# anonymous-author-918/deq-mpc-corl

Hardware: AMD Instinct MI355X
Metric: QP solves/sec at (B,T=20,nx=13,nu=4) (higher is better)
Workload: dtype f32

## Files before the change

### deq-mpc-corl_amd/csrc/alqp_quad.hip

```cpp
#include <hip/hip_runtime.h>

#include "alqp_quad.hpp"
#include "alqp_dims.hpp"
#include "alqp_launch.hpp"

#if defined(ALQP_QUAD_F32) == defined(ALQP_QUAD_F64)
#error "compile alqp_quad.hip with exactly one of -DALQP_QUAD_F32, -DALQP_QUAD_F64"
#endif

namespace alqp {

#ifndef ALQP_FUSE_LS
#define ALQP_FUSE_LS 1
#endif
#ifdef ALQP_PHASE_TIMING
__device__ unsigned long long g_phase_cycles[10];
#define QSTAMP(b) qd.stamp(b)
#else
#define QSTAMP(b)
#endif
template <typename real, int NX, int NU, bool TRACE, class Dyn = NoDyn>
__global__ __launch_bounds__(64) __attribute__((amdgpu_waves_per_eu(1, 1))) void k_solve_lin_quad(SolveArgs<real> a, TraceArgs<real> tr, real *ws) {
    using C = QCfg<real, NX, NU>;
    constexpr bool NL = Dyn::ID != 0;
// ... 19 lines not shown
            if (mode == 4) simd = (simd & 1) ^ (blockIdx.x & 1);
            if (mode == 5) simd = (hw >> 8) & 3;
            for (int i = 0; i < simd * stag; ++i) __builtin_amdgcn_s_sleep(16);
        }
    }
#ifdef ALQP_ALIAS_ALL
    const int b = (active ? b_raw : a.B - 1) % ALQP_ALIAS_ALL;
#else
    const int b = active ? b_raw : a.B - 1;
#endif
    const int T = a.T, M = C::M(T);

    Quad<real, NX, NU> qd;
    __shared__ real w_lds[QCfg<real, NX, NU>::WLDS_WORDS];
    qd.wl = w_lds + threadIdx.x;
    qd.q = lane & 3;
    qd.T = T;
    qd.active = active;
    qd.gQd = a.Qd + (size_t)b * T * N;
    qd.gq = a.q + (size_t)b * T * N;
    qd.gF = a.F + (size_t)b * (T - 1) * NX * N;
    qd.gc = a.c + (size_t)b * (T - 1) * NX;
    qd.gx0 = a.x0 + (size_t)b * NX;
    qd.gulo = a.ulo + (size_t)b * a.sb_u;
    qd.guhi = a.uhi + (size_t)b * a.sb_u;
    qd.st_u = a.st_u;
    qd.gz = a.z + (size_t)b * T * N;
    qd.glam = a.lam + (size_t)b * M;
    qd.rec = ws + C::rec_base(b, T);
    qd.gFw = const_cast<real *>(qd.gF);
    qd.dyn_h = a.dyn_h;
    qd.rho = a.rho[b];
    qd.info = 0;
    real phi_prev = a.phi[b];
#ifdef ALQP_PHASE_TIMING
    for (int i = 0; i < 10; ++i) qd.tacc[i] = 0;
#endif
    QSTAMP(-1);
    if (!(a.flags & ALQP_WS_PRIMED)) {
        if constexpr (NL) qd.stage_in(false, false);
        else qd.stage_in(a.max_newton == 0 || a.al_iter == 0 || (a.flags & ALQP_EXIT_IN_KERNEL) ||
                         (!C::PHI0_FWD && (a.flags & ALQP_INIT_MERIT)));
    }
    const bool ref_exit = (a.flags & ALQP_EXIT_IN_KERNEL) != 0;
    int gphase = 0;

    int step_id = 0;
    bool pend = false;
    real alpha_pend = 0;
    int bad = 0;
    real rn2 = 0, phi_next = 0;
    for (int it = 0; it < a.al_iter; ++it) {
        bool phi_from_forward = false;
        if (a.flags & ALQP_INIT_MERIT) {
            if (it > 0) {
                phi_prev = phi_next;
            } else if (C::PHI0_FWD && a.max_newton > 0 && !ref_exit) {
                phi_from_forward = true;
            } else {
                if constexpr (NL) qd.template linearize<Dyn>(real(0), false);
                real p1[1];
                qd.template merit_candidates<1>(p1, true);
                phi_prev = p1[0];
            }
        }
        pend = false;
        double nrm_old = 0;
        int n_done = 0;
        if (ref_exit) {
            int bad0 = 0;
            const real r0 = it == 0 ? qd.rplus2(bad0) : rn2;
            nrm_old = sqrt(grid_sum_ordered(wave_sum_leaders(exit_term(r0, qor(qd.info)), active && qd.q == 0), a.exit_scratch, gphase));
        }
        for (int st = 0; st < a.max_newton; ++st, ++step_id) {
            real *tg = nullptr;
            if constexpr (TRACE) tg = (tr.g && active) ? tr.g + ((size_t)step_id * a.B + b) * T * N : nullptr;
            QSTAMP(9);
            if constexpr (NL) {
                qd.template linearize<Dyn>(alpha_pend, pend);
                pend = false;
            }
            qd.forward(tg, alpha_pend, pend, (phi_from_forward && st == 0) ? &phi_prev : nullptr);
            real ph[20];
            qd.template backward<FUSE_LS>(ph);
            QSTAMP(-1);
            if constexpr (TRACE) {
                if (tr.d && active) {
                    real *td = tr.d + ((size_t)step_id * a.B + b) * T * N;
                    for (int t = 0; t < T; ++t)
                        for (int j = qd.q; j < N; j += 4) td[t * N + j] = qd.recp(t)[C::wn(C::oY, j)];
                }
            }
            if constexpr (NL) qd.template merit_nonlin<Dyn>(ph);
            else if constexpr (!FUSE_LS) qd.template merit_candidates<20>(ph, false);
            QSTAMP(6);
            int kbest = 0;
            real best = ph[0];
#pragma unroll
            for (int k = 1; k < 20; ++k) {
                if (k < a.n_ls && !(best != best) && (ph[k] != ph[k] || ph[k] < best)) {
                    best = ph[k];
                    kbest = k;
                }
            }
            const bool acc = best < phi_prev;
            if constexpr (TRACE) {
                if (active && qd.q == 0) {
                    if (tr.phi)
#pragma unroll
                        for (int k = 0; k < 20; ++k)
                            if (k < a.n_ls) tr.phi[((size_t)step_id * a.n_ls + k) * a.B + b] = ph[k];
                    if (tr.phi_prev) tr.phi_prev[(size_t)step_id * a.B + b] = phi_prev;
                    if (tr.k) tr.k[(size_t)step_id * a.B + b] = kbest;
                    if (tr.accept) tr.accept[(size_t)step_id * a.B + b] = acc ? 1 : 0;
                }
            }
            const real alpha = acc ? real(1) / real(1 << kbest) : real(0);
            pend = true;
            alpha_pend = alpha;
            QSTAMP(7);
            phi_prev = best;
            if (ref_exit) {
                int bad1 = 0;
                real ph_unused = 0, r1 = 0;
                qd.template iter_end<Dyn>(alpha_pend, pend, false, (real)a.rho_scale, false, ph_unused, r1, bad1);
                pend = false;
                const double nw = sqrt(grid_sum_ordered(wave_sum_leaders(exit_term(r1, qor(qd.info)), active && qd.q == 0), a.exit_scratch, gphase));
                ++n_done;
                if (nw < a.exit_tol || fabs(nrm_old - nw) / nw < a.exit_tol) break;
                nrm_old = nw;
            }
        }
        if (ref_exit && a.newton_counts && blockIdx.x == 0 && lane == 0) a.newton_counts[it] = grid_barrier_timed_out(a.exit_scratch) ? -1 : n_done;
        bad = 0;
        qd.template iter_end<Dyn>(alpha_pend, pend, (a.flags & ALQP_DUAL_UPDATE) != 0, (real)a.rho_scale, it + 1 == a.al_iter,
                    phi_next, rn2, bad);
        pend = false;
    }
    if (a.al_iter <= 0) {
        rn2 = qd.rplus2(bad);
        qd.stage_out();
    }
#ifdef ALQP_PHASE_TIMING
    QSTAMP(9);
    if (lane == 0)
        for (int i = 0; i < 10; ++i) atomicAdd(&g_phase_cycles[i], qd.tacc[i]);
#endif
    if (active && qd.q == 0) {
        a.rho[b] = qd.rho;
        a.phi[b] = phi_prev;
        if (a.rnorm2) a.rnorm2[b] = rn2;
        if (a.info && qd.info && a.info[b] == 0) a.info[b] = qd.info;
        if (a.status) a.status[b] = bad ? 0 : 1;
    }
}

template <typename real, int NX, int NU>
__global__ __launch_bounds__(64) __attribute__((amdgpu_waves_per_eu(1, 1))) void k_backward_quad(BwdArgs<real> a, real *ws) {
    using C = QCfg<real, NX, NU>;
    constexpr int N = C::N;
    const int lane = threadIdx.x, qi = lane >> 2;
    const int b_raw = blockIdx.x * 16 + qi;
    const bool active = b_raw < a.B;
    const int b = active ? b_raw : a.B - 1;
    const int T = a.T;
    Quad<real, NX, NU> qd;
    __shared__ real w_lds[QCfg<real, NX, NU>::WLDS_WORDS];
    qd.wl = w_lds + threadIdx.x;
    qd.q = lane & 3;
    qd.T = T;
    qd.active = active;
    qd.gF = a.F + (size_t)b * (T - 1) * NX * N;
    qd.gQd = nullptr; qd.gq = nullptr; qd.gc = nullptr; qd.gx0 = nullptr; qd.gulo = nullptr; qd.guhi = nullptr;
    qd.st_u = 0;
    qd.gz = nullptr; qd.glam = nullptr;
    qd.rec = ws + C::rec_base(b, T);
    qd.rho = a.rho[b];
    qd.info = 0;
    qd.solve_forward(a.gbar + (size_t)b * T * N);
    real unused[20];
    qd.template backward<false>(unused);
    if (active) {
        const real *zf = a.z_final + (size_t)b * T * N;
        real *qg = a.q_grad + (size_t)b * T * N;
        real *Qg = a.Qd_grad + (size_t)b * T * N;
        for (int t = 0; t < T; ++t)
            for (int j = qd.q; j < N; j += 4) {
                const real w = qd.recp(t)[C::wn(C::oY, j)];
                qg[t * N + j] = w;
                Qg[t * N + j] = w * zf[t * N + j];
            }
    }
}

template <typename real, int NX, int NU>
__global__ __launch_bounds__(64) __attribute__((amdgpu_waves_per_eu(1, 1))) void k_newton_step_quad(StepArgs<real> a, real *ws) {
    using C = QCfg<real, NX, NU>;
    constexpr int N = C::N, SW = C::SW;
    const int lane = threadIdx.x, qi = lane >> 2;
    const int b_raw = blockIdx.x * 16 + qi;
    const bool active = b_raw < a.B;
    const int b = active ? b_raw : a.B - 1;
    const int T = a.T, M = C::M(T) + T * a.nobs;
    Quad<real, NX, NU> qd;
    __shared__ real w_lds[QCfg<real, NX, NU>::WLDS_WORDS];
    qd.wl = w_lds + threadIdx.x;
    qd.q = lane & 3;
    qd.T = T;
    qd.active = active;
    qd.gQd = a.Qd + (size_t)b * T * N;
    qd.gq = a.q + (size_t)b * T * N;
    qd.gF = a.F + (size_t)b * (T - 1) * NX * N;
    qd.gc = nullptr;
    qd.gx0 = a.x0 + (size_t)b * NX;
    qd.gulo = a.ulo + (size_t)b * a.sb_u;
    qd.guhi = a.uhi + (size_t)b * a.sb_u;
    qd.st_u = a.st_u;
    qd.gz = const_cast<real *>(a.z) + (size_t)b * T * N;
    qd.glam = const_cast<real *>(a.lam) + (size_t)b * M;
    qd.rec = ws + C::rec_base(b, T);
    qd.gFw = const_cast<real *>(qd.gF);
    qd.dyn_h = 0;
    qd.rho = a.rho[b];
    qd.info = 0;
    qd.nobs = a.nobs;
    qd.gobs = a.nobs > 0 ? a.obs + (size_t)b * T * a.nobs * 3 : nullptr;
    qd.obs_r2 = a.obs_r2;
    qd.no_init = a.no_init != 0;
    const real *gxn = a.xnext + (size_t)b * (T - 1) * NX;
    real *tg = (a.g_out && active) ? a.g_out + (size_t)b * T * N : nullptr;
    qd.template forward<true>(tg, real(0), false, nullptr, gxn);
    real unused[20];
    qd.template backward<false>(unused, a.d_out + (size_t)b * T * N);
    if (active) {
        if (qd.q == 0 && a.info && qd.info && a.info[b] == 0) a.info[b] = qd.info;
    }
}


template <typename real, int NX, int NU, typename Fn, typename... Args>
int launch_quad_kernel(Fn fn, int B, hipStream_t stream, Args... args) {
    const unsigned grid = (unsigned)((B + 15) / 16);
    return launch_maybe_coop(fn, grid, 0, stream, args...);
}

template <typename real>
int dispatch_solve_quad(int nx, int nu, const SolveArgs<real> &a, const TraceArgs<real> *tr, real *ws,
                        hipStream_t stream) {
    return for_dims(nx, nu, ALQP_E_UNSUPPORTED, [&](auto NX, auto NU) {
        if (tr) return launch_quad_kernel<real, NX, NU>(k_solve_lin_quad<real, NX, NU, true>, a.B, stream, a, *tr, ws);
        return launch_quad_kernel<real, NX, NU>(k_solve_lin_quad<real, NX, NU, false>, a.B, stream, a, TraceArgs<real>{}, ws);
    });
}

template <typename real>
int dispatch_backward_quad(int nx, int nu, const BwdArgs<real> &a, real *ws, hipStream_t stream) {
    return for_dims(nx, nu, ALQP_E_UNSUPPORTED, [&](auto NX, auto NU) {
        return launch_quad_kernel<real, NX, NU>(k_backward_quad<real, NX, NU>, a.B, stream, a, ws);
    });
}

template <typename real>
int dispatch_solve_nonlin(int dyn_id, int nx, int nu, const SolveArgs<real> &a, real *ws, hipStream_t stream) {
    if (dyn_id == DynPendulum1l<real>::ID && nx == 2 && nu == 1)
        return launch_quad_kernel<real, 2, 1>(k_solve_lin_quad<real, 2, 1, false, DynPendulum1l<real>>, a.B, stream, a,
                                              TraceArgs<real>{}, ws);
    if (dyn_id == DynCartpole1l<real>::ID && nx == 4 && nu == 1)
        return launch_quad_kernel<real, 4, 1>(k_solve_lin_quad<real, 4, 1, false, DynCartpole1l<real>>, a.B, stream, a,
                                              TraceArgs<real>{}, ws);
    if (dyn_id == DynCartpole1l<real, 2>::ID && nx == 4 && nu == 1)
        return launch_quad_kernel<real, 4, 1>(k_solve_lin_quad<real, 4, 1, false, DynCartpole1l<real, 2>>, a.B, stream, a,
                                              TraceArgs<real>{}, ws);
    if (dyn_id == DynCartpole2l<real>::ID && nx == 6 && nu == 1)
        return launch_quad_kernel<real, 6, 1>(k_solve_lin_quad<real, 6, 1, false, DynCartpole2l<real>>, a.B, stream, a,
                                              TraceArgs<real>{}, ws);
    return ALQP_E_UNSUPPORTED;
}

template <typename real>
int dispatch_step_quad(int nx, int nu, const StepArgs<real> &a, real *ws, hipStream_t stream) {
    return for_dims(nx, nu, ALQP_E_UNSUPPORTED, [&](auto NX, auto NU) {
        return launch_quad_kernel<real, NX, NU>(k_newton_step_quad<real, NX, NU>, a.B, stream, a, ws);
    });
}

#ifdef ALQP_QUAD_F32
using quad_real = float;
#else
using quad_real = double;
#endif
template int dispatch_solve_quad<quad_real>(int, int, const SolveArgs<quad_real> &, const TraceArgs<quad_real> *, quad_real *, hipStream_t);
template int dispatch_backward_quad<quad_real>(int, int, const BwdArgs<quad_real> &, quad_real *, hipStream_t);
template int dispatch_solve_nonlin<quad_real>(int, int, int, const SolveArgs<quad_real> &, quad_real *, hipStream_t);
template int dispatch_step_quad<quad_real>(int, int, const StepArgs<quad_real> &, quad_real *, hipStream_t);

}

#if defined(ALQP_PHASE_TIMING) && defined(ALQP_QUAD_F32)
extern "C" int alqp_debug_phase_cycles(unsigned long long *out10, int reset) {
    if (out10 && hipMemcpyFromSymbol(out10, HIP_SYMBOL(alqp::g_phase_cycles), 10 * sizeof(unsigned long long)) != hipSuccess) return -1;
    if (reset) {
        unsigned long long z[10] = {0};
        if (hipMemcpyToSymbol(HIP_SYMBOL(alqp::g_phase_cycles), z, sizeof(z)) != hipSuccess) return -1;
    }
    return 0;
}
#endif
```

### deq-mpc-corl_amd/csrc/alqp_quad.hpp

```cpp
#pragma once
#include <hip/hip_runtime.h>

#include <type_traits>

#include "alqp_team.hpp"
#include "alqp_dyn.hpp"

namespace alqp {

template <int Q>
__device__ inline float qb(float v) {
    return __builtin_bit_cast(float, __builtin_amdgcn_mov_dpp(__builtin_bit_cast(int, v), Q * 0x55, 0xF, 0xF, true));
}
template <int Q>
__device__ inline double qb(double v) {
    long long b = __builtin_bit_cast(long long, v);
    int lo = __builtin_amdgcn_mov_dpp((int)(b & 0xffffffffll), Q * 0x55, 0xF, 0xF, true);
    int hi = __builtin_amdgcn_mov_dpp((int)(b >> 32), Q * 0x55, 0xF, 0xF, true);
    return __builtin_bit_cast(double, ((long long)hi << 32) | (unsigned int)lo);
}
template <typename real>
__device__ inline real qbv(real v, int src) {
    switch (src & 3) {
        case 0: return qb<0>(v);
// ... 68 lines not shown
#ifndef ALQP_EXP_NOL
#define ALQP_EXP_NOL 0
#endif
template <typename real, int SW, int N, bool IN_LDS>
struct WPanel {
    real a[SW][N];
    __device__ __forceinline__ real (&operator[](int s))[N] { return a[s]; }
    __device__ __forceinline__ const real (&operator[](int s) const)[N] { return a[s]; }
};
template <typename real, int N>
struct WRowLds {
    real *p;
    __device__ __forceinline__ real &operator[](int k) const { return p[k * 64]; }
};
template <typename real, int SW, int N>
struct WPanel<real, SW, N, true> {
    real *base;
    __device__ __forceinline__ WRowLds<real, N> operator[](int s) const { return WRowLds<real, N>{base + s * N * 64}; }
};
template <int LEN, typename real>
__device__ __forceinline__ void gload(const real *p, WRowLds<real, LEN> row) {
    real tmp[LEN];
    gload<LEN>(p, tmp);
#pragma unroll
    for (int k = 0; k < LEN; ++k) row[k] = tmp[k];
}

struct NoDyn {
    static constexpr int ID = 0;
};

struct Fld {
    int h, t;
};
template <int H, int T>
struct FldT {
    static constexpr int h = H, t = T;
    __host__ __device__ constexpr operator Fld() const { return {H, T}; }
};
template <typename real>
struct FRef {
    real *p;
    Fld f;
};
template <typename real, int H, int T>
__device__ __forceinline__ FRef<std::remove_const_t<real>> operator+(real *p, FldT<H, T>) {
    return {const_cast<std::remove_const_t<real> *>(p), Fld{H, T}};
}

template <typename real, int NX_, int NU_>
struct QCfg {
    static constexpr int NX = NX_, NU = NU_, N = NX_ + NU_;
    static constexpr int SH = (N + 3) / 4;
    static constexpr int SW = (NX + 3) / 4;
    static constexpr int SY = SH;
    static constexpr int HT = 2 * SH * (SH + 1);
    __host__ __device__ static constexpr int hidx(int s, int j) { return 2 * s * (s + 1) + j; }
    static constexpr int ST = 2 * SW * (SW + 1);
    static constexpr int BLK = 64 / (int)sizeof(real);
#ifndef ALQP_REC_IL_F32
#define ALQP_REC_IL_F32 2
#endif
    static constexpr int IL = sizeof(real) == 4 ? ALQP_REC_IL_F32 : 1;
    static_assert(IL == 1 || BLK == 16, "groups of 16 words are 64-byte blocks");
    __host__ __device__ static constexpr int w(int x) { return (x / 16) * (16 * IL) + x % 16; }
    static constexpr int NLAST = N - 4 * (SH - 1);
    __host__ __device__ static constexpr int lanes_of(int s) { return s == SH - 1 ? NLAST : 4; }
    __host__ __device__ static constexpr int lstride(int s) { return lanes_of(s) == 3 ? 16 : 4 * lanes_of(s); }
    __host__ __device__ static constexpr int lbase(int s) {
        int o = 0;
        for (int i = 0; i < s; ++i) o += (i + 1) * lstride(i);
        return o;
    }
    static constexpr int LW = lbase(SH);
    static constexpr bool PHI0_FWD = sizeof(real) == 4;
#ifndef ALQP_S_AFTER_F32
#define ALQP_S_AFTER_F32 0
#endif
    static constexpr bool S_AFTER = sizeof(real) == 8 || ALQP_S_AFTER_F32;
#ifndef ALQP_W_LDS_F32
#define ALQP_W_LDS_F32 0
#endif
    static constexpr bool W_LDS = ALQP_W_LDS && (sizeof(real) == 8 || ALQP_W_LDS_F32);
    static constexpr int WLDS_WORDS = W_LDS ? SW * N * 64 : 1;
    __host__ __device__ static constexpr int p4(int x) { return (x + 3) & ~3; }
    static constexpr int NF = 9;
    __host__ __device__ static constexpr int fslots(int i) { return (i <= 1 || i == 6 || i == 7) ? SY : (i == 5 ? 4 : SW); }
    static constexpr int oL = 2 * 16 * (SY / 4);
    __host__ __device__ static constexpr int tail_at(int i) {
        int g = (oL + LW + 15) & ~15, o = 0;
        for (int k = 0; k < NF; ++k) {
            const int r = fslots(k) % 4;
            if (r > 0 && o + r > 4) { g += 16; o = 0; }
            if (k == i) return g + o;
            o += r;
        }
        return o > 0 ? g + 16 : g;
    }
    __host__ __device__ static constexpr int head_at(int i) {
        if (i < 2) return i * 16 * (SY / 4);
        int o = tail_at(NF);
        for (int k = 2; k < i; ++k) o += 16 * (fslots(k) / 4);
        return o;
    }
    static constexpr FldT<head_at(0), tail_at(0)> oY{};
    static constexpr FldT<head_at(1), tail_at(1)> oZ{};
    static constexpr FldT<head_at(2), tail_at(2)> oR{};
    static constexpr FldT<head_at(3), tail_at(3)> oS{};
    static constexpr FldT<head_at(4), tail_at(4)> oLE{};
    static_assert(NU <= 4, "the u-slot layout holds one control per lane");
    static constexpr FldT<head_at(5), tail_at(5)> oUS{};
    static constexpr FldT<head_at(6), tail_at(6)> oQ{};
    static constexpr FldT<head_at(7), tail_at(7)> oq{};
    static constexpr FldT<head_at(8), tail_at(8)> oC{};
    static constexpr int RECW = (head_at(NF) + 31) & ~31;
    static_assert(IL == 1 || RECW % 16 == 0, "whole groups per record");
    template <int S>
    __host__ __device__ static constexpr int lp(int m, int q) {
        return m < 4 * (S / 4) ? 16 * (m / 4) + 4 * q + m % 4 : 16 * (S / 4) + q * (S % 4) + m - 4 * (S / 4);
    }
    template <int S>
    __host__ __device__ static constexpr int fw(Fld f, int p) {
        return p < 16 * (S / 4) ? w(f.h + p) : w(f.t + 4 * ((p - 16 * (S / 4)) / (S % 4)) + (p - 16 * (S / 4)) % (S % 4));
    }
    __host__ __device__ static constexpr int pn(int k) { return lp<SY>(k >> 2, k & 3); }
    __host__ __device__ static constexpr int px(int r) { return lp<SW>(r >> 2, r & 3); }
    __host__ __device__ static constexpr int wn(Fld f, int k) { return fw<SY>(f, pn(k)); }
    __host__ __device__ static constexpr int M(int T) { return T * NX + 2 * T * NU; }
    static constexpr int RSTR = RECW * IL;
    __host__ __device__ static constexpr size_t rec_base(int b, int T) { return (size_t)(b / IL) * T * RSTR + (size_t)(b % IL) * 16; }
    __host__ __device__ static constexpr size_t ws_words(int B, int T) { return (size_t)((B + IL - 1) / IL) * T * RSTR; }
    __host__ static bool ws_covers(int B, int T) {
        return rec_base(B - 1, T) + (size_t)(T - 1) * RSTR + w(RECW - 1) + 1 <= ws_words(B, T);
    }
};

template <typename real, int NX, int NU>
struct Quad {
    using C = QCfg<real, NX, NU>;
    static constexpr int N = C::N, SH = C::SH, SW = C::SW, SY = C::SY, HT = C::HT, ST = C::ST, RECW = C::RECW;

    int q, T;
    bool active;
    const real *gQd, *gq, *gF, *gc, *gx0, *gulo, *guhi;
    long st_u;
    real *gz, *glam, *rec;
    real rho;
    int info;
    real *wl;
    using WT = WPanel<real, SW, N, C::W_LDS>;
    __device__ __forceinline__ WT wpanel() const {
        if constexpr (C::W_LDS) return WT{wl};
        else return WT{};
    }
    real *gFw;
    real dyn_h;
    const real *gobs;
    int nobs;
    real obs_r2;
    bool no_init;

    __device__ __forceinline__ real uhi(int t, int j) const { return guhi[t * st_u + j]; }
    __device__ __forceinline__ real ulo(int t, int j) const { return gulo[t * st_u + j]; }
    __device__ __forceinline__ real *recp(int t) const { return rec + (size_t)t * C::RSTR; }
#ifdef ALQP_PHASE_TIMING
    unsigned long long tacc[10], tlast;
    __device__ __forceinline__ void stamp(int bucket) {
// ... 57 lines not shown
        for (int c = (LEN / 4) * 4; c < LEN; ++c) p[c] = v[c];
    }
    __device__ __forceinline__ void st_own_n(FRef<real> f, const real (&v)[SY]) const { st_slots<SY>(f, v); }
    __device__ __forceinline__ void st_own_x(FRef<real> f, const real (&v)[SW]) const { st_slots<SW>(f, v); }
    __device__ __forceinline__ void ld_rep_n(FRef<real> f, real (&v)[N]) const {
        real w[4 * SY];
        ld_field<SY>(f, w);
#pragma unroll
        for (int k = 0; k < N; ++k) v[k] = w[C::pn(k)];
    }
    __device__ __forceinline__ void ld_repx_of_n(FRef<real> f, real (&v)[NX]) const {
        real w[4 * SY];
        ld_field<SY>(f, w);
#pragma unroll
        for (int k = 0; k < NX; ++k) v[k] = w[C::pn(k)];
    }
    __device__ __forceinline__ void ld_rep_x(FRef<real> f, real (&v)[NX]) const {
        real w[4 * SW];
        ld_field<SW>(f, w);
#pragma unroll
        for (int r = 0; r < NX; ++r) v[r] = w[C::px(r)];
    }
    __device__ __forceinline__ real *lchunk(real *rp, int s, int c, int ql) const {
        return rp + C::w(C::oL + C::lbase(s) + c * C::lstride(s)) + 4 * ql;
    }
    template <int LEN, int SL>
    __device__ __forceinline__ void own_of(const real (&full)[LEN], real (&v)[SL]) const {
#pragma unroll
        for (int m = 0; m < SL; ++m)
            v[m] = (4 * m < LEN) ? sel4(full[(4 * m < LEN) ? 4 * m : 0], (4 * m + 1 < LEN) ? full[(4 * m + 1 < LEN) ? 4 * m + 1 : 0] : real(0),
                                        (4 * m + 2 < LEN) ? full[(4 * m + 2 < LEN) ? 4 * m + 2 : 0] : real(0),
                                        (4 * m + 3 < LEN) ? full[(4 * m + 3 < LEN) ? 4 * m + 3 : 0] : real(0), q)
                                 : real(0);
    }
    template <int LEN, int SL>
    __device__ __forceinline__ void ld_own_ext(const real *src, real (&v)[SL]) const {
#pragma unroll
        for (int m = 0; m < SL; ++m) {
            const int k = 4 * m + q;
            const real x = src[(4 * m + 3 < LEN || k < LEN) ? k : LEN - 1];
            v[m] = (4 * m + 3 < LEN || k < LEN) ? x : real(0);
        }
    }
    template <int LEN, int SL>
    __device__ __forceinline__ void st_own_ext(real *dst, const real (&v)[SL]) const {
#pragma unroll
        for (int m = 0; m < SL; ++m)
            if (4 * m + 3 < LEN || 4 * m + q < LEN) dst[4 * m + q] = v[m];
    }

    __device__ __forceinline__ int own_ju() const { return (q - NX) & 3; }
    __device__ __forceinline__ void ld_own_us(const real *rp, real &lu, real &ll, real &bu, real &bl) const {
        gld4(rp + C::w(C::oUS.h) + 4 * q, lu, ll, bu, bl);
    }
    __device__ __forceinline__ void st_own_us(real *rp, real lu, real ll, real bu, real bl) const {
        gst4(rp + C::w(C::oUS.h) + 4 * q, lu, ll, bu, bl);
    }
    __device__ __forceinline__ void ld_rep_us(const real *rp, real (&lu)[NU], real (&ll)[NU], real (&bu)[NU], real (&bl)[NU]) const {
        real w[16];
        ld_field<4>(rp + C::oUS, w);
#pragma unroll
        for (int ju = 0; ju < NU; ++ju) {
            const int ql = (NX + ju) & 3;
            lu[ju] = w[4 * ql];
            ll[ju] = w[4 * ql + 1];
            bu[ju] = w[4 * ql + 2];
            bl[ju] = w[4 * ql + 3];
        }
    }

    __device__ __forceinline__ void load_F_rows(int t, WT &W) const {
        const real *Fg = gF + (size_t)t * NX * N;
#pragma unroll
        for (int s = 0; s < SW; ++s) {
            const int r = 4 * s + q;
            const int rc = (4 * s + 3 < NX) ? r : (r < NX ? r : NX - 1);
            gload<N>(Fg + rc * N, W[s]);
            if (4 * s + 3 >= NX) {
                const real m = r < NX ? real(1) : real(0);
#pragma unroll
                for (int k = 0; k < N; ++k) W[s][k] *= m;
            }
        }
    }
    template <int LEN>
    __device__ __forceinline__ void copy_slice(const real *src, real *dst) const {
#pragma unroll
        for (int c = 0; 16 * c < LEN; ++c) {
            const int w0 = 16 * c + 4 * q;
            if (16 * c + 15 < LEN || w0 + 3 < LEN) {
                real a, b, cc, d;
                gld4(src + w0, a, b, cc, d);
                gst4(dst + w0, a, b, cc, d);
            } else {
#pragma unroll
                for (int w = 0; w < 4; ++w)
                    if (w0 + w < LEN) dst[w0 + w] = src[w0 + w];
            }
        }
    }
    __device__ __forceinline__ void stage_in(bool with_residual, bool have_c = true) {
#pragma unroll 2
        for (int t = 0; t < T; ++t) {
            const bool dyn = t < T - 1;
            real *rp = recp(t);
            if (active) {
                real vn[SY], vx[SW];
                ld_own_ext<N>(gz + t * N, vn);
                st_own_n(rp + C::oZ, vn);
                ld_own_ext<N>(gQd + t * N, vn);
                st_own_n(rp + C::oQ, vn);
                ld_own_ext<N>(gq + t * N, vn);
                st_own_n(rp + C::oq, vn);
                ld_own_ext<NX>(glam + t * NX, vx);
                st_own_x(rp + C::oLE, vx);
                {
                    const int ju = own_ju(), jc = ju < NU ? ju : 0;
                    const real *lb = glam + T * NX + t * 2 * NU;
                    const real a0 = lb[jc], a1 = lb[NU + jc], a2 = guhi[t * st_u + jc], a3 = gulo[t * st_u + jc];
                    const bool has = ju < NU;
                    st_own_us(rp, has ? a0 : real(0), has ? a1 : real(0), has ? a2 : real(0), has ? a3 : real(0));
                }
                if (dyn && have_c) ld_own_ext<NX>(gc + t * NX, vx);
                else {
#pragma unroll
                    for (int s = 0; s < SW; ++s) vx[s] = 0;
                }
                if (have_c) st_own_x(rp + C::oC, vx);
            }
            if (with_residual) {
                WT W = wpanel();
                real zt[N];
                load_F_rows(dyn ? t : (T > 1 ? T - 2 : 0), W);
                gload<N>(gz + t * N, zt);
                real rr[SW];
#pragma unroll
                for (int s = 0; s < SW; ++s) {
                    const int r = 4 * s + q;
                    rr[s] = 0;
                    if (4 * s + 3 < NX || r < NX) {
                        real xn = dyn ? gc[t * NX + r] : real(0);
#pragma unroll
                        for (int k = 0; k < N; ++k) xn = fma_(W[s][k], zt[k], xn);
                        rr[s] = dyn ? gz[(t + 1) * N + r] - xn : gz[r] - gx0[r];
                    }
                }
                if (active) st_own_x(rp + C::oR, rr);
            }
        }
    }
    __device__ __forceinline__ void stage_out() {
        if (!active) return;
#pragma unroll 2
        for (int t = 0; t < T; ++t) {
            const real *rp = recp(t);
            real vn[SY], vx[SW];
            ld_own_n(rp + C::oZ, vn);
            st_own_ext<N>(gz + t * N, vn);
            ld_own_x(rp + C::oLE, vx);
            st_own_ext<NX>(glam + t * NX, vx);
            {
                real lu, ll, bu, bl;
                ld_own_us(rp, lu, ll, bu, bl);
                const int ju = own_ju();
                if (ju < NU) {
                    glam[T * NX + t * 2 * NU + ju] = lu;
// ... 393 lines not shown
                            for (int s = 0; s < SW; ++s)
                                if (k0 + kk < N) wv[kk][s] = W[s][k0 + kk];
                        __builtin_amdgcn_sched_barrier(0);
#pragma unroll
                        for (int kk = 0; kk < KB; ++kk) {
                            const int k = k0 + kk;
                            if (k < N) {
                                const real lkj = qbv(H[C::hidx(k >> 2, j)], k) * ip;
#pragma unroll
                                for (int s = (k >> 2); s < SH; ++s) H[C::hidx(s, k)] = fma_(-H[C::hidx(s, j)], lkj, H[C::hidx(s, k)]);
#pragma unroll
                                for (int s = 0; s < SW; ++s) W[s][k] = fma_(-wj[s], lkj, wv[kk][s]);
                                Y[k] = fma_(-Y[j], lkj, Y[k]);
                            }
                        }
                    }
                } else {
#pragma unroll
                for (int k = j + 1; k < N; ++k) {
                    const real lkj = qbv(H[C::hidx(k >> 2, j)], k) * ip;
#pragma unroll
                    for (int s = (k >> 2); s < SH; ++s) H[C::hidx(s, k)] = fma_(-H[C::hidx(s, j)], lkj, H[C::hidx(s, k)]);
#pragma unroll
                    for (int s = 0; s < SW; ++s) W[s][k] = fma_(-W[s][j], lkj, W[s][k]);
                    Y[k] = fma_(-Y[j], lkj, Y[k]);
                }
                }
                if constexpr (C::S_AFTER) ipv[j] = ip;
                if (!C::S_AFTER && dyn) {
#pragma unroll
                    for (int b = 0; b < NX; ++b) {
                        const real wbj = qbv(W[b >> 2][j], b) * ip;
#pragma unroll
                        for (int s = (b >> 2); s < SW; ++s) S[C::hidx(s, b)] = fma_(W[s][j], wbj, S[C::hidx(s, b)]);
                    }
                    const real yip = Y[j] * ip;
#pragma unroll
                    for (int s = 0; s < SW; ++s) Sy[s] = fma_(W[s][j], yip, Sy[s]);
                }
                H[C::hidx(j >> 2, j)] = (q == (j & 3)) ? ip : H[C::hidx(j >> 2, j)];
            }
            ALQP_STAMP(2);
            if (active) {
                if (!(ALQP_EXP_NOL && t >= T - ALQP_EXP_NOL))
#pragma unroll
                for (int s = 0; s < SH; ++s)
#pragma unroll
                    for (int c = 0; c <= s; ++c)
                        if (C::lanes_of(s) == 4 || q < C::lanes_of(s))
                            gst4(lchunk(rp, s, c, q), H[C::hidx(s, 4 * c)],
                                 H[C::hidx(s, 4 * c + 1)], H[C::hidx(s, 4 * c + 2)], H[C::hidx(s, 4 * c + 3)]);
                real yo[SY];
                own_of<N, SY>(Y, yo);
                st_own_n(rp + C::oY, yo);
                if (pending) st_own_n(rp + C::oZ, zs);
            }

            if constexpr (C::S_AFTER) {
                if (dyn) {
#pragma unroll
                    for (int j = 0; j < N; ++j) {
#pragma unroll
                        for (int b = 0; b < NX; ++b) {
                            const real wbj = qbv(W[b >> 2][j], b) * ipv[j];
#pragma unroll
                            for (int s = (b >> 2); s < SW; ++s) S[C::hidx(s, b)] = fma_(W[s][j], wbj, S[C::hidx(s, b)]);
                        }
                        const real yip = Y[j] * ipv[j];
#pragma unroll
                        for (int s = 0; s < SW; ++s) Sy[s] = fma_(W[s][j], yip, Sy[s]);
                    }
                }
            }
#pragma unroll
            for (int s = 0; s < SW; ++s) {
                vpo[s] = v[s];
                Syo[s] = Sy[s];
            }
            ALQP_STAMP(3);
        }
        if constexpr (C::PHI0_FWD) { if (phi0) *phi0 = qsum(mdist); }
    }

    template <bool LS>
    __device__ __forceinline__ void backward(real (&phi)[20], real *d_ext = nullptr) {
        constexpr int MU0 = NX / 4;
        real c0 = 0, c1 = 0, c2 = 0;
        real acc[20];
        real rvT[SW], lvT[SW];
#pragma unroll
        for (int k = 0; k < 20; ++k) acc[k] = 0;
#pragma unroll
        for (int s = 0; s < SW; ++s) rvT[s] = lvT[s] = 0;
        real dxn[NX];
#pragma unroll
        for (int j = 0; j < NX; ++j) dxn[j] = 0;
        for (int t = T - 1; t >= 0; --t) {
            const bool dyn = t < T - 1;
            real *rp = recp(t);
            real H[HT];
            if (ALQP_EXP_NOL && t >= T - ALQP_EXP_NOL) {
#pragma unroll
                for (int i = 0; i < HT; ++i) H[i] = real(1);
            } else
#pragma unroll
            for (int s = 0; s < SH; ++s)
#pragma unroll
                for (int c = 0; c <= s; ++c) {
                    const int ql = (C::lanes_of(s) == 4 || q < C::lanes_of(s)) ? q : 0;
                    gld4(lchunk(rp, s, c, ql), H[C::hidx(s, 4 * c)],
                         H[C::hidx(s, 4 * c + 1)], H[C::hidx(s, 4 * c + 2)], H[C::hidx(s, 4 * c + 3)]);
                }
            real yo[SY];
            ld_own_n(rp + C::oY, yo);
            real Y[N];
#pragma unroll
            for (int j = 0; j < N; ++j) Y[j] = qbv(yo[j >> 2], j);
            WT W = wpanel();
            load_F_rows(dyn ? t : (T > 1 ? T - 2 : 0), W);
            real zz[SY], QQ[SY], qq[SY], rv[SW], lv[SW];
            real lu = 0, ll = 0, bu = 0, bl = 0;
            if constexpr (LS) {
                ld_own_n(rp + C::oZ, zz);
                if constexpr (ALQP_EXP_NOQ) { for (int m = 0; m < SY; ++m) QQ[m] = real(1); }
                else ld_own_n(rp + C::oQ, QQ);
                ld_own_n(rp + C::oq, qq);
                ld_own_us(rp, lu, ll, bu, bl);
                if constexpr (ALQP_EXP_NORS) { for (int s = 0; s < SW; ++s) rv[s] = real(0); }
                else ld_own_x(rp + C::oR, rv);
                ld_own_x(rp + C::oLE, lv);
            }
            ALQP_STAMP(4);
            real dxs[SW];
#pragma unroll
            for (int s = 0; s < SW; ++s)
                dxs[s] = sel4(dxn[4 * s], (4 * s + 1 < NX) ? dxn[(4 * s + 1 < NX) ? 4 * s + 1 : 0] : real(0),
                              (4 * s + 2 < NX) ? dxn[(4 * s + 2 < NX) ? 4 * s + 2 : 0] : real(0),
                              (4 * s + 3 < NX) ? dxn[(4 * s + 3 < NX) ? 4 * s + 3 : 0] : real(0), q);
            if (dyn) {
                real vv[N];
#pragma unroll
                for (int j = 0; j < N; ++j) {
                    real p = 0;
#pragma unroll
                    for (int s = 0; s < SW; ++s) p = fma_(W[s][j], dxs[s], p);
                    vv[j] = qsum(p);
                }
#pragma unroll
                for (int j = 0; j < N; ++j) {
                    const real wj = vv[j] * qbv(H[C::hidx(j >> 2, j)], j);
#pragma unroll
                    for (int k = j + 1; k < N; ++k) vv[k] = fma_(-qbv(H[C::hidx(k >> 2, j)], k), wj, vv[k]);
                }
#pragma unroll
                for (int j = 0; j < N; ++j) Y[j] = fma_(rho, vv[j], Y[j]);
            }
#pragma unroll
            for (int i = N - 1; i >= 0; --i) {
                const real di = Y[i] * qbv(H[C::hidx(i >> 2, i)], i);
                Y[i] = di;
#pragma unroll
                for (int j = 0; j < i; ++j) Y[j] = fma_(-qbv(H[C::hidx(i >> 2, j)], i), di, Y[j]);
            }
            if (active) {
                real down[SY];
                own_of<N, SY>(Y, down);
// ... 382 lines not shown
```

Before: 5.984 million.

## Add software-pipelined fp32 backward sweep that prefetches next stage's F and factor rows

Adds a backward_pipe variant of the Riccati-style backward sweep that double-buffers the next time step's F rows, y values and Cholesky factor chunks, issuing their global loads while the current step computes. An accvgpr read and sched barriers are used to force the loads to be in flight across the stage boundary. By default it runs for the plain (non-line-search) backward in the solve, gradient and newton-step kernels for fp32. The line-search fused version stays off unless a macro enables it. This hides global-load latency in the sequential time loop, at the cost of roughly doubled register pressure for the buffered sets.

Result: no change. 5.991 million (median of 5 runs) (+0.1%).

```diff
diff --git a/deq-mpc-corl_amd/csrc/alqp_quad.hip b/deq-mpc-corl_amd/csrc/alqp_quad.hip
--- a/deq-mpc-corl_amd/csrc/alqp_quad.hip
+++ b/deq-mpc-corl_amd/csrc/alqp_quad.hip
@@ -125,7 +125,8 @@
             }
             qd.forward(tg, alpha_pend, pend, (phi_from_forward && st == 0) ? &phi_prev : nullptr);
             real ph[20];
-            qd.template backward<FUSE_LS>(ph);
+            if constexpr (FUSE_LS ? C::BWD_PIPE_LS : C::BWD_PIPE_PLAIN) qd.template backward_pipe<FUSE_LS>(ph);
+            else qd.template backward<FUSE_LS>(ph);
             QSTAMP(-1);
             if constexpr (TRACE) {
                 if (tr.d && active) {
@@ -222,7 +223,8 @@
     qd.info = 0;
     qd.solve_forward(a.gbar + (size_t)b * T * N);
     real unused[20];
-    qd.template backward<false>(unused);
+    if constexpr (C::BWD_PIPE_PLAIN) qd.template backward_pipe<false>(unused);
+    else qd.template backward<false>(unused);
     if (active) {
         const real *zf = a.z_final + (size_t)b * T * N;
         real *qg = a.q_grad + (size_t)b * T * N;
@@ -274,7 +276,8 @@
     real *tg = (a.g_out && active) ? a.g_out + (size_t)b * T * N : nullptr;
     qd.template forward<true>(tg, real(0), false, nullptr, gxn);
     real unused[20];
-    qd.template backward<false>(unused, a.d_out + (size_t)b * T * N);
+    if constexpr (C::BWD_PIPE_PLAIN) qd.template backward_pipe<false>(unused, a.d_out + (size_t)b * T * N);
+    else qd.template backward<false>(unused, a.d_out + (size_t)b * T * N);
     if (active) {
         if (qd.q == 0 && a.info && qd.info && a.info[b] == 0) a.info[b] = qd.info;
     }
diff --git a/deq-mpc-corl_amd/csrc/alqp_quad.hpp b/deq-mpc-corl_amd/csrc/alqp_quad.hpp
--- a/deq-mpc-corl_amd/csrc/alqp_quad.hpp
+++ b/deq-mpc-corl_amd/csrc/alqp_quad.hpp
@@ -174,7 +174,18 @@
 #define ALQP_W_LDS_F32 0
 #endif
     static constexpr bool W_LDS = ALQP_W_LDS && (sizeof(real) == 8 || ALQP_W_LDS_F32);
-    static constexpr int WLDS_WORDS = W_LDS ? SW * N * 64 : 1;
+#ifndef ALQP_BWD_PIPE
+#define ALQP_BWD_PIPE 1
+#endif
+    static constexpr bool BWD_PIPE_OK = ALQP_BWD_PIPE && sizeof(real) == 4 && !W_LDS && !ALQP_EXP_NOQ && !ALQP_EXP_NORS && !ALQP_EXP_NOL;
+    static constexpr bool BWD_PIPE_PLAIN = BWD_PIPE_OK;
+#ifndef ALQP_BWD_PIPE_LS
+#define ALQP_BWD_PIPE_LS 0
+#endif
+    static constexpr bool BWD_PIPE_LS = BWD_PIPE_OK && ALQP_BWD_PIPE_LS;
+    static constexpr bool BWD_LDS = BWD_PIPE_LS;
+    static constexpr int BWD_LDS_WORDS = BWD_LDS ? (20 + 2 * SW) * 64 : 1;
+    static constexpr int WLDS_WORDS = W_LDS ? SW * N * 64 : BWD_LDS_WORDS;
     __host__ __device__ static constexpr int p4(int x) { return (x + 3) & ~3; }
     static constexpr int NF = 9;
     __host__ __device__ static constexpr int fslots(int i) { return (i <= 1 || i == 6 || i == 7) ? SY : (i == 5 ? 4 : SW); }
@@ -398,6 +409,24 @@
                 for (int k = 0; k < N; ++k) W[s][k] *= m;
             }
         }
+    }
+    __device__ __forceinline__ void load_F_rows_raw(int t, WT &W) const {
+        const real *Fg = gF + (size_t)t * NX * N;
+#pragma unroll
+        for (int s = 0; s < SW; ++s) {
+            const int r = 4 * s + q;
+            const int rc = (4 * s + 3 < NX) ? r : (r < NX ? r : NX - 1);
+            gload<N>(Fg + rc * N, W[s]);
+        }
+    }
+    __device__ __forceinline__ void mask_F_rows(WT &W) const {
+#pragma unroll
+        for (int s = 0; s < SW; ++s)
+            if (4 * s + 3 >= NX) {
+                const real m = 4 * s + q < NX ? real(1) : real(0);
+#pragma unroll
+                for (int k = 0; k < N; ++k) W[s][k] *= m;
+            }
     }
     template <int LEN>
     __device__ __forceinline__ void copy_slice(const real *src, real *dst) const {
@@ -957,6 +986,240 @@
         if constexpr (C::PHI0_FWD) { if (phi0) *phi0 = qsum(mdist); }
     }
 
+    struct BwdSet {
+        WT W;
+        real yo[SY];
+        real H[HT];
+    };
+    __device__ __forceinline__ void bwd_load(int t, BwdSet &s) const {
+        t = t < 0 ? 0 : (t > T - 1 ? T - 1 : t);
+        const real *rp = recp(t);
+        load_F_rows_raw(t < T - 1 ? t : (T > 1 ? T - 2 : 0), s.W);
+        ld_own_n(const_cast<real *>(rp) + C::oY, s.yo);
+#pragma unroll
+        for (int sl = 0; sl < SH; ++sl)
+#pragma unroll
+            for (int c = 0; c <= sl; ++c) {
+                const int ql = (C::lanes_of(sl) == 4 || q < C::lanes_of(sl)) ? q : 0;
+                const real *p = lchunk(const_cast<real *>(rp), sl, c, ql);
+                if (4 * c + 3 < N) gld4(p, s.H[C::hidx(sl, 4 * c)], s.H[C::hidx(sl, 4 * c + 1)], s.H[C::hidx(sl, 4 * c + 2)], s.H[C::hidx(sl, 4 * c + 3)]);
+                else
+#pragma unroll
+                    for (int i = 0; 4 * c + i < N; ++i) s.H[C::hidx(sl, 4 * c + i)] = p[i];
+            }
+    }
+    __device__ __forceinline__ static float acc_read(float x) {
+        float r;
+        asm("v_accvgpr_read_b32 %0, %1" : "=v"(r) : "a"(x));
+        return r;
+    }
+    __device__ __forceinline__ void bwd_take(BwdSet &s) const {
+        static_assert(sizeof(real) == 4, "the pipelined sweep is fp32 only");
+#pragma unroll
+        for (int sl = 0; sl < SW; ++sl)
+#pragma unroll
+            for (int k = 0; k < N; ++k) s.W[sl][k] = acc_read(s.W[sl][k]);
+#pragma unroll
+        for (int m = 0; m < SY; ++m) s.yo[m] = acc_read(s.yo[m]);
+#pragma unroll
+        for (int sl = 0; sl < SH; ++sl)
+#pragma unroll
+            for (int j = 0; j < 4 * sl + 4; ++j)
+                if (j < N) s.H[C::hidx(sl, j)] = acc_read(s.H[C::hidx(sl, j)]);
+    }
+    template <int LEN, bool IN_LDS>
+    struct LaneArr {
+        real a[LEN];
+        __device__ __forceinline__ LaneArr(real *) {}
+        __device__ __forceinline__ real get(int k) const { return a[k]; }
+        __device__ __forceinline__ void set(int k, real v) { a[k] = v; }
+    };
+    template <int LEN>
+    struct LaneArr<LEN, true> {
+        real *p;
+        __device__ __forceinline__ LaneArr(real *p_) : p(p_) {}
+        __device__ __forceinline__ real get(int k) const { return p[64 * k]; }
+        __device__ __forceinline__ void set(int k, real v) { p[64 * k] = v; }
+    };
+    template <bool LS>
+    __device__ __forceinline__ void backward_pipe(real (&phi)[20], real *d_ext = nullptr) {
+        static_assert(!C::W_LDS, "the pipelined sweep keeps both sets of F rows in registers");
+        constexpr int MU0 = NX / 4;
+        constexpr bool CL = LS && C::BWD_LDS;
+        asm volatile("" : "+v"(q));
+        {
+            int z0 = 0;
+            asm volatile("" : "+v"(z0));
+            rec += z0;
+            gF += z0;
+        }
+        LaneArr<20, CL> acc(wl);
+        LaneArr<SW, CL> rvT(wl + 20 * 64), lvT(wl + (20 + SW) * 64);
+        real c0 = 0, c1 = 0, c2 = 0;
+        real dxs[SW];
+        if constexpr (LS) {
+#pragma unroll
+            for (int k = 0; k < 20; ++k) acc.set(k, real(0));
+#pragma unroll
+            for (int s = 0; s < SW; ++s) { rvT.set(s, real(0)); lvT.set(s, real(0)); }
+        }
+#pragma unroll
+        for (int s = 0; s < SW; ++s) dxs[s] = 0;
+        auto stage = [&](const int t, BwdSet &cur, BwdSet &nxt) __attribute__((always_inline)) {
+            const bool dyn = t < T - 1;
+            real *rp = recp(t);
+            real zz[SY], QQ[SY], qq[SY], rv[SW], lv[SW];
+            real lu = 0, ll = 0, bu = 0, bl = 0;
+            if constexpr (LS) {
+                ld_own_n(rp + C::oZ, zz);
+                ld_own_n(rp + C::oQ, QQ);
+                ld_own_n(rp + C::oq, qq);
+                ld_own_us(rp, lu, ll, bu, bl);
+                ld_own_x(rp + C::oR, rv);
+                ld_own_x(rp + C::oLE, lv);
+                __builtin_amdgcn_sched_barrier(0);
+            }
+            bwd_take(cur);
+            __builtin_amdgcn_sched_barrier(0);
+            bwd_load(t - 1, nxt);
+            __builtin_amdgcn_sched_barrier(0);
+            mask_F_rows(cur.W);
+            real Y[N];
+#pragma unroll
+            for (int j = 0; j < N; ++j) Y[j] = qbv(cur.yo[j >> 2], j);
+            if (dyn) {
+                real vv[N];
+#pragma unroll
+                for (int j = 0; j < N; ++j) {
+                    real p = 0;
+#pragma unroll
+                    for (int s = 0; s < SW; ++s) p = fma_(cur.W[s][j], dxs[s], p);
+                    vv[j] = qsum(p);
+                }
+#pragma unroll
+                for (int j = 0; j < N; ++j) {
+                    const real wj = vv[j] * qbv(cur.H[C::hidx(j >> 2, j)], j);
+#pragma unroll
+                    for (int k = j + 1; k < N; ++k) vv[k] = fma_(-qbv(cur.H[C::hidx(k >> 2, j)], k), wj, vv[k]);
+                }
+#pragma unroll
+                for (int j = 0; j < N; ++j) Y[j] = fma_(rho, vv[j], Y[j]);
+            }
+#pragma unroll
+            for (int i = N - 1; i >= 0; --i) {
+                const real di = Y[i] * qbv(cur.H[C::hidx(i >> 2, i)], i);
+                Y[i] = di;
+#pragma unroll
+                for (int j = 0; j < i; ++j) Y[j] = fma_(-qbv(cur.H[C::hidx(i >> 2, j)], i), di, Y[j]);
+            }
+            if (active) {
+                real down[SY];
+                own_of<N, SY>(Y, down);
+                if (d_ext) st_own_ext<N>(d_ext + t * N, down);
+                else st_own_n(rp + C::oY, down);
+            }
+            real sv[SW];
+#pragma unroll
+            for (int s = 0; s < SW; ++s) sv[s] = 0;
+            if (dyn) {
+#pragma unroll
+                for (int s = 0; s < SW; ++s) {
+                    const int r = 4 * s + q;
+                    real p = 0;
+#pragma unroll
+                    for (int k = 0; k < N; ++k) p = fma_(cur.W[s][k], Y[k], p);
+                    sv[s] = (4 * s + 3 < NX || r < NX) ? dxs[s] - p : real(0);
+                }
+                if (active && !d_ext) st_own_x(rp + C::oS, sv);
+            }
+            if constexpr (LS) {
+                real zu = 0, du = 0;
+#pragma unroll
+                for (int m = 0; m < SY; ++m) {
+                    const int j = 4 * m + q;
+                    const real ok = (4 * m + 3 < N || j < N) ? real(1) : real(0);
+                    const real dj = sel4(Y[4 * m], (4 * m + 1 < N) ? Y[(4 * m + 1 < N) ? 4 * m + 1 : 0] : real(0),
+                                         (4 * m + 2 < N) ? Y[(4 * m + 2 < N) ? 4 * m + 2 : 0] : real(0),
+                                         (4 * m + 3 < N) ? Y[(4 * m + 3 < N) ? 4 * m + 3 : 0] : real(0), q);
+                    const real z = zz[m], d = dj * ok, Qv = QQ[m] * ok, qv = qq[m] * ok;
+                    c0 = fma_(fma_(real(0.5) * Qv, z, qv), z, c0);
+                    c1 = fma_(fma_(Qv, z, qv), d, c1);
+                    c2 = fma_(real(0.5) * Qv * d, d, c2);
+                    if (m >= MU0) {
+                        const bool mine = j >= NX && j < N;
+                        zu = mine ? z : zu;
+                        du = mine ? d : du;
+                    }
+                }
+                {
+                    const real isu = own_ju() < NU ? real(1) : real(0);
+                    real alpha = 1;
+#pragma unroll
+                    for (int k = 0; k < 20; ++k) {
+                        real zk = fma_(alpha, du, zu);
+                        real vu = zk - bu, vl = bl - zk;
+                        real cu = fmax_(vu, real(0)), cl = fmax_(vl, real(0));
+                        acc.set(k, fma_(isu, fma_(lu, vu, ll * vl) + real(0.5) * rho * fma_(cu, cu, cl * cl), acc.get(k)));
+                        alpha *= real(0.5);
+                    }
+                }
+                if (dyn) {
+#pragma unroll
+                    for (int s = 0; s < SW; ++s) {
+                        const int r = 4 * s + q;
+                        const real ok = (4 * s + 3 < NX || r < NX) ? real(1) : real(0);
+                        const real rr = rv[s] * ok, ss = sv[s] * ok, lm = lv[s] * ok;
+                        c0 = fma_(fma_(real(0.5) * rho, rr, lm), rr, c0);
+                        c1 = fma_(fma_(rho, rr, lm), ss, c1);
+                        c2 = fma_(real(0.5) * rho * ss, ss, c2);
+                    }
+                } else {
+#pragma unroll
+                    for (int s = 0; s < SW; ++s) {
+                        rvT.set(s, rv[s]);
+                        lvT.set(s, lv[s]);
+                    }
+                }
+            }
+#pragma unroll
+            for (int s = 0; s < SW; ++s)
+                dxs[s] = sel4(Y[4 * s], (4 * s + 1 < NX) ? Y[(4 * s + 1 < NX) ? 4 * s + 1 : 0] : real(0),
+                              (4 * s + 2 < NX) ? Y[(4 * s + 2 < NX) ? 4 * s + 2 : 0] : real(0),
+                              (4 * s + 3 < NX) ? Y[(4 * s + 3 < NX) ? 4 * s + 3 : 0] : real(0), q);
+            ALQP_STAMP(5);
+        };
+        BwdSet A, Bs;
+        bwd_load(T - 1, A);
+        ALQP_STAMP(4);
+        int t = T - 1;
+        for (; t >= 1; t -= 2) {
+            stage(t, A, Bs);
+            stage(t - 1, Bs, A);
+        }
+        if (t == 0) stage(0, A, Bs);
+        if (active && !d_ext) st_own_x(recp(T - 1) + C::oS, dxs);
+        if constexpr (LS) {
+#pragma unroll
+            for (int s = 0; s < SW; ++s) {
+                const int r = 4 * s + q;
+                const real ok = (4 * s + 3 < NX || r < NX) ? real(1) : real(0);
+                const real rr = rvT.get(s) * ok, ss = dxs[s] * ok, lm = lvT.get(s) * ok;
+                c0 = fma_(fma_(real(0.5) * rho, rr, lm), rr, c0);
+                c1 = fma_(fma_(rho, rr, lm), ss, c1);
+                c2 = fma_(real(0.5) * rho * ss, ss, c2);
+            }
+            c0 = qsum(c0);
+            c1 = qsum(c1);
+            c2 = qsum(c2);
+            real alpha = 1;
+#pragma unroll
+            for (int k = 0; k < 20; ++k) {
+                phi[k] = qsum(acc.get(k)) + fma_(alpha, fma_(alpha, c2, c1), c0);
+                alpha *= real(0.5);
+            }
+        }
+    }
+
     template <bool LS>
     __device__ __forceinline__ void backward(real (&phi)[20], real *d_ext = nullptr) {
         constexpr int MU0 = NX / 4;
```
